# Antibas/eaQHM-analysis-and-synthesis-in-Python

Hardware: AMD Instinct MI355X
Metric: analysis_frames_per_sec (higher is better)
Workload: dtype f64; 1 GPU; synth16k_60s_female_maxAdpt5; samples=960000, fs=16000, ls_frames_per_adaptation=63936, adaptations_executed=5, Kmax=59, track_bytes=906240000, parallelism=instants sharded x1 by LS cost; boundary records all-gathered per adaptation

## Files before the change

eaqhm-analysis-and-synthesis-in-python_amd/csrc/eaqhm_ls_tile.hip:

```cpp
#include "eaqhm_ls_common.h"
#include "eaqhm_ls_chol.h"
#include "eaqhm_ls_a0.h"
#include "eaqhm_ls_tilemap.h"

namespace eaqhm {


#define DIAG_OWNER(jb, nt) ((int)TL_DIAG[nt][jb])
#define TL_THREADS 512
#define TL_WAVES 8
#define TL_CW 8
#define TL_NTMAX 13
#define CI_STRIDE 20
#define CI_NCH 16
#define A0_NS 7
#define A0_M 7

#define TZ_TB 104
#define TZ_NCH 8

__device__ inline void tw_step(d4 (&g)[9], double aR, double aI, double bR, double bI, double nk) {
  const double sA = aR + aI, dB = bI - bR;
  const double naR = nk * aR, naI = nk * aI, nsA = nk * sA;
  const double nbR = nk * bR, nbI = nk * bI, ndB = nk * dB;
  g[0] = __builtin_amdgcn_mfma_f64_16x16x4f64(aR, bR, g[0], 0, 0, 0);
  g[1] = __builtin_amdgcn_mfma_f64_16x16x4f64(aI, bI, g[1], 0, 0, 0);
  g[2] = __builtin_amdgcn_mfma_f64_16x16x4f64(sA, dB, g[2], 0, 0, 0);
  g[3] = __builtin_amdgcn_mfma_f64_16x16x4f64(naR, bR, g[3], 0, 0, 0);
  g[4] = __builtin_amdgcn_mfma_f64_16x16x4f64(naI, bI, g[4], 0, 0, 0);
  g[5] = __builtin_amdgcn_mfma_f64_16x16x4f64(nsA, dB, g[5], 0, 0, 0);
  g[6] = __builtin_amdgcn_mfma_f64_16x16x4f64(naR, nbR, g[6], 0, 0, 0);
  g[7] = __builtin_amdgcn_mfma_f64_16x16x4f64(naI, nbI, g[7], 0, 0, 0);
  g[8] = __builtin_amdgcn_mfma_f64_16x16x4f64(nsA, ndB, g[8], 0, 0, 0);
}

template <int NS, int TW>
__device__ __attribute__((noinline)) void tile_frame(const LsArgs& A, int TS_, int ldx_max_, double* lds, int f_) {
  const int TS = uni(TS_), ldx_max = uni(ldx_max_), f = uni(f_);
  const int tid = threadIdx.x, nt_thr = TL_THREADS;
  const int lane = tid & 63;
  const int wave = __builtin_amdgcn_readfirstlane(tid >> 6);
  double* U = uni(lds);
  double* Xre = U;
  double* Xim = Xre + (size_t)TS * ldx_max;
  const size_t usize_g = (size_t)2 * TS * ldx_max;
  double* ci = U + usize_g;
  unsigned long long* masks = (unsigned long long*)(ci + (size_t)CI_STRIDE * 52);
  double* PanR = U;
  double* PanI = PanR + TL_NTMAX * TL_TILE;
  double* WtR = PanI + TL_NTMAX * TL_TILE;
  double* WtI = WtR + TL_NTMAX * TL_TILE;
  double* LdR = WtI + TL_NTMAX * TL_TILE;
  double* LdI = LdR + TL_TILE;
  double* Dc = LdI + TL_TILE;
  double* Zc = Dc + DG_TILE;
  double* zv = Zc + DG_TILE;
  double* xv = zv + 2 * 16 * TL_NTMAX;
  const size_t usize_c = (size_t)(xv + 32 - U);
  double* xs = U + usize_c;
  double* sh = xs + 4 * uni(A.Kcmax);
  double* win = sh + 16;
  double* sig = win + 64 * CI_NCH;
  double* dorig = sig + 64 * CI_NCH;

  const int Npad = ((uni(A.Nmax) + 63) >> 6) << 6;
  double* Qs = uni(A.scratch) + (size_t)blockIdx.x * (size_t)uni((int)A.scratch_stride);
  double* Rs = Qs + (size_t)Npad * uni(A.nmax);
  const bool seeds = uni((int)(A.any_seed && (*A.any_seed != 0))) != 0;
  const double w1 = uni(2.0 * M_PI / A.fs);
  const int PE = TS / 2;
  const double* sA = uni(A.s);
  const int lcol = lane & 15, lq = lane >> 4;
  unsigned long long* dbg = uni(A.debug);
  unsigned long long t_prev = 0;

  {
    const int n = uni(A.ncol[f]);
    const int Kc = 2 * n + 1, Ms = 2 * Kc + 1;
    const int nt = (Ms + 15) >> 4;
    const int c = uni(A.frame_c[f]), wl = uni(A.frame_wl[f]), inst = uni(A.frame_inst[f]);
    const int N = 2 * wl + 1, mid = wl;
    const int T = (Kc + 16) >> 4;
    const int nb = TW ? T : nt;
    const int ldx = (nb << 4) + ((nb & 1) ? 0 : 16);
    const int npair = T * (T + 1) / 2;
    const int is = 2 * Kc - 16 * (nt - 1);
    const double f0 = uni(A.f0_stale);
    const int* mycols = uni(A.cols) + (size_t)f * uni(A.Kmax);
    const int npairs = mid + 1;

    if (dbg && tid == 0) t_prev = __builtin_amdgcn_s_memtime();
    for (int q = tid; q < 2 * TS * ldx_max; q += nt_thr) Xre[q] = 0.0;
    for (int t = tid; t < N; t += nt_thr) {
      win[t] = window_value(false, t, N);
      sig[t] = sA[(size_t)(c - wl) + t];
    }
    __syncthreads();
    int* gappy = (int*)(masks + (size_t)52 * CI_NCH);
    prepare_slots<CI_STRIDE, TL_WAVES>(A, Qs, Rs, Npad, ci, masks, gappy, mycols, n, N, mid, c, wl, seeds, lane, wave, CI_NCH);
    LS_STAMP(0);

    constexpr int NM3 = (NS <= 7) ? NS : 0;
    d4 accR[NS], accI[NS], acc3[NM3 ? NM3 : 1];
    int tP[NS], tQ[NS];
    bool live[NS];
#pragma unroll
    for (int sl = 0; sl < NS; ++sl) {
      accR[sl] = (d4){0, 0, 0, 0};
      accI[sl] = (d4){0, 0, 0, 0};
      if (sl < NM3) acc3[sl] = (d4){0, 0, 0, 0};
      const int code = TL_MAP[nt][wave][sl];
      live[sl] = code != 0xFF;
      const int P = live[sl] ? (code >> 4) : 0, Q = live[sl] ? (code & 15) : 0;
      tP[sl] = __builtin_amdgcn_readfirstlane(P);
      tQ[sl] = __builtin_amdgcn_readfirstlane(Q);
    }

    constexpr int TWA = TW ? TW : 1;
    d4 g[TWA][9];
    int gI[TWA], gJ[TWA];
    bool glive[TWA];
#pragma unroll
    for (int sl = 0; sl < TWA; ++sl) {
      const int x = wave + 8 * sl;
      glive[sl] = TW && x < npair;
      int I = 0, J = 0;
      if (glive[sl]) tile_of(x, I, J);
      gI[sl] = __builtin_amdgcn_readfirstlane(I);
      gJ[sl] = __builtin_amdgcn_readfirstlane(J);
#pragma unroll
      for (int p = 0; p < 9; ++p) g[sl][p] = (d4){0, 0, 0, 0};
    }

    for (int d0 = 0; d0 < npairs; d0 += PE) {
#pragma clang loop unroll(disable)
      for (int idx = tid; idx < 16 * n; idx += nt_thr) {
        const int el = idx & 15, j = idx >> 4, d = d0 + el;
        const bool act = d <= mid;
        const int u = mid - d - 1, v = mid + d;
        double su = 0, cu = 1, sv, cv;
        double pur = 0, pui = 0, nur = 0, nui = 0, pvr, pvi, nvr, nvi;
        {
          double* cj = ci + j * CI_STRIDE;
          const double* fb = ((const double**)cj)[2];
          const double* ab = ((const double**)cj)[3];
          const int dc = act ? d : mid;
          const double fu1 = fb[mid - dc], fv = fb[mid + dc];
          const double au = ab[(mid - dc - 1 >= 0) ? (mid - dc - 1) : 0], au1 = ab[mid - dc];
          const double av = ab[mid + dc], av1 = ab[(mid + dc + 1 < N) ? (mid + dc + 1) : (N - 1)];
          const double xu = act ? fu1 : 0.0, xv = (act && d >= 1) ? fv : 0.0;
          const double qv = cj[0] + scan16(xv), qu = -(cj[1] + scan16(xu));
          if (el == 15) { cj[0] = qv; cj[1] = -qu; }
          if (!act) continue;
          const double ainv = cj[17], pr = cj[18], pi = cj[19];
          sincos_cw(qu * w1, &su, &cu);
          sincos_cw(qv * w1, &sv, &cv);
          const double eps = 10e-5;
          if (u >= 0) {
            const double ru = (eps + au) * ainv, rv1 = (eps + av1) * ainv;
            pur = ru * cu;                    pui = ru * su;
            nur = rv1 * (cv * pr - sv * pi);  nui = rv1 * (cv * pi + sv * pr);
          }
          const double rv = (eps + av) * ainv, ru1 = (eps + au1) * ainv;
          pvr = rv * cv;                      pvi = rv * sv;
          nvr = ru1 * (cu * pr - su * pi);    nvi = ru1 * (cu * pi + su * pr);
        }
        double* xr = Xre + (2 * el) * ldx;
        double* xi = Xim + (2 * el) * ldx;
        const int cpos = XCOL(n + 1 + j, el), cneg = XCOL(j, el);
        const int spos = XCOL(Kc + n + 1 + j, el), sneg = XCOL(Kc + j, el);
        const double wv = win[v], nv = (double)(v - mid);
        if (u >= 0) {
          const double wu = win[u], nu = (double)(u - mid);
          pur *= wu; pui *= wu; nur *= wu; nui *= wu;
          xr[cpos] = pur;      xi[cpos] = pui;      xr[cneg] = nur;      xi[cneg] = nui;
          if (!TW) { xr[spos] = nu * pur; xi[spos] = nu * pui; xr[sneg] = nu * nur; xi[sneg] = nu * nui; }
        }
        pvr *= wv; pvi *= wv; nvr *= wv; nvi *= wv;
        xr += ldx; xi += ldx;
        xr[cpos] = pvr;      xi[cpos] = pvi;      xr[cneg] = nvr;      xi[cneg] = nvi;
        if (!TW) { xr[spos] = nv * pvr; xi[spos] = nv * pvi; xr[sneg] = nv * nvr; xi[sneg] = nv * nvi; }
      }
      if ((tid & 15) == 0 && (tid >> 4) < TS) {
        const int row = tid >> 4;
        const int d = d0 + (row >> 1);
        const int t = (row & 1) ? (mid + d) : (mid - d - 1);
        const bool ok = (d <= mid) && (t >= 0);
        const double w = ok ? win[t] : 0.0;
        const double sval = ok ? sig[t] : 0.0;
        const double nn = (double)(t - mid);
        const int el = row >> 1;
        double* xr = Xre + row * ldx;
        double* xi = Xim + row * ldx;
        xr[XCOL(n, el)] = w;               xi[XCOL(n, el)] = 0.0;
        if (!TW) {
          xr[XCOL(Kc + n, el)] = w * nn;   xi[XCOL(Kc + n, el)] = 0.0;
        }
        const int scol = TW ? Kc : 2 * Kc;
        xr[XCOL(scol, el)] = w * sval;     xi[XCOL(scol, el)] = 0.0;
      }
      if (d0 + PE > mid) {
        for (int q = tid; q < TS * 16 * nb; q += nt_thr) {
          const int row = q / (16 * nb), col = q - row * (16 * nb);
          const int d = d0 + (row >> 1);
          const int t = (row & 1) ? (mid + d) : (mid - d - 1);
          if (d > mid || t < 0) { Xre[row * ldx + col] = 0.0; Xim[row * ldx + col] = 0.0; }
        }
      }
      LS_STAMP(12);
      __syncthreads();
      LS_STAMP(1);
      const int pcs = (npairs - d0 < PE) ? (npairs - d0) : PE;
      const int ksl = (pcs + 1) >> 1;
      if constexpr (TW > 0) {
#pragma unroll
        for (int sl = 0; sl < TW; ++sl) {
          if (!glive[sl]) continue;
          const int ca = 16 * gI[sl], cb = 16 * gJ[sl];
          int rb = lq * ldx;
          const int sw0 = lcol + (lq >> 1);
          int nk = (lq & 1) ? d0 + (lq >> 1) : -d0 - (lq >> 1) - 1;
          asm volatile("" : "+v"(rb), "+v"(nk));
          const int plane = TS * ldx_max;
          const int kn = (ksl < 8) ? ksl : 8;
#pragma clang loop unroll(disable)
          for (int ks = 0; ks < kn; ++ks) {
            const int sw = (sw0 + 2 * ks) & 15;
            const double aR = Xre[rb + ca + sw], aI = Xre[rb + ca + sw + plane];
            const double bR = Xre[rb + cb + sw], bI = Xre[rb + cb + sw + plane];
            rb += 4 * ldx;
            tw_step(g[sl], aR, aI, bR, bI, (double)nk);
            nk += (lq & 1) ? 2 : -2;
          }
        }
      } else
#pragma unroll
      for (int sl = 0; sl < NS; ++sl) {
        if (!live[sl]) continue;
        const int ca = 16 * tP[sl], cb = 16 * tQ[sl];
        int rb = lq * ldx;
        const int sw0 = lcol + (lq >> 1);
        asm volatile("" : "+v"(rb));
        const int plane = TS * ldx_max;
        if (ksl < 8) {
#pragma clang loop unroll(disable)
          for (int ks = 0; ks < ksl; ++ks) {
            const int sw = (sw0 + 2 * ks) & 15;
            const double aR = Xre[rb + ca + sw], aI = Xre[rb + ca + sw + plane];
            const double bR = Xre[rb + cb + sw], bI = Xre[rb + cb + sw + plane];
            rb += 4 * ldx;
            if (sl < NM3) {
              accR[sl] = __builtin_amdgcn_mfma_f64_16x16x4f64(aR, bR, accR[sl], 0, 0, 0);
              acc3[sl < NM3 ? sl : 0] = __builtin_amdgcn_mfma_f64_16x16x4f64(aI, bI, acc3[sl < NM3 ? sl : 0], 0, 0, 0);
              accI[sl] = __builtin_amdgcn_mfma_f64_16x16x4f64(aR + aI, bI - bR, accI[sl], 0, 0, 0);
            } else {
              accR[sl] = __builtin_amdgcn_mfma_f64_16x16x4f64(aR, bR, accR[sl], 0, 0, 0);
              accI[sl] = __builtin_amdgcn_mfma_f64_16x16x4f64(aR, bI, accI[sl], 0, 0, 0);
              accR[sl] = __builtin_amdgcn_mfma_f64_16x16x4f64(aI, bI, accR[sl], 0, 0, 0);
              accI[sl] = __builtin_amdgcn_mfma_f64_16x16x4f64(-aI, bR, accI[sl], 0, 0, 0);
            }
          }
          continue;
        }
        double aR, aI, bR, bI;
        {
          const int sw = sw0 & 15;
          aR = Xre[rb + ca + sw]; aI = Xre[rb + ca + sw + plane]; bR = Xre[rb + cb + sw]; bI = Xre[rb + cb + sw + plane];
        }
#pragma unroll
        for (int ks = 0; ks < 8; ++ks) {
          double naR = 0, naI = 0, nbR = 0, nbI = 0;
          if (ks < 7) {
            rb += 4 * ldx;
            const int sw = (sw0 + 2 * (ks + 1)) & 15;
            naR = Xre[rb + ca + sw]; naI = Xre[rb + ca + sw + plane]; nbR = Xre[rb + cb + sw]; nbI = Xre[rb + cb + sw + plane];
          }
          __builtin_amdgcn_sched_barrier(0);
          if (sl < NM3) {
            accR[sl] = __builtin_amdgcn_mfma_f64_16x16x4f64(aR, bR, accR[sl], 0, 0, 0);
            acc3[sl < NM3 ? sl : 0] = __builtin_amdgcn_mfma_f64_16x16x4f64(aI, bI, acc3[sl < NM3 ? sl : 0], 0, 0, 0);
            accI[sl] = __builtin_amdgcn_mfma_f64_16x16x4f64(aR + aI, bI - bR, accI[sl], 0, 0, 0);
          } else {
            accR[sl] = __builtin_amdgcn_mfma_f64_16x16x4f64(aR, bR, accR[sl], 0, 0, 0);
            accI[sl] = __builtin_amdgcn_mfma_f64_16x16x4f64(aR, bI, accI[sl], 0, 0, 0);
            accR[sl] = __builtin_amdgcn_mfma_f64_16x16x4f64(aI, bI, accR[sl], 0, 0, 0);
            accI[sl] = __builtin_amdgcn_mfma_f64_16x16x4f64(-aI, bR, accI[sl], 0, 0, 0);
          }
          aR = naR; aI = naI; bR = nbR; bI = nbI;
        }
      }
      __syncthreads();
      LS_STAMP(2);
    }
    if constexpr (TW == 0 && NM3 > 0) {
#pragma unroll
      for (int sl = 0; sl < NM3; ++sl) {
        const d4 p1 = accR[sl], p2 = acc3[sl];
        accR[sl] = p1 + p2;
        accI[sl] = accI[sl] + (p1 - p2);
      }
    }
    if constexpr (TW > 0) {
      double* Gs = Qs;
#pragma unroll
      for (int sl = 0; sl < TWA; ++sl) {
        if (!glive[sl]) continue;
        const int x = wave + 8 * sl;
#pragma unroll
        for (int p = 0; p < 3; ++p) {
          const d4 p1 = g[sl][3 * p], p2 = g[sl][3 * p + 1];
          const d4 re = p1 + p2, im = g[sl][3 * p + 2] + (p1 - p2);
          double* gt = Gs + (size_t)(p * npair + x) * 512;
#pragma unroll
          for (int r = 0; r < 4; ++r) {
            const int o = 2 * (16 * (lq + 4 * r) + lcol);
            gt[o] = re[r]; gt[o + 1] = im[r];
          }
        }
      }
      __syncthreads();
#pragma unroll
      for (int sl = 0; sl < NS; ++sl) {
#pragma unroll
        for (int r = 0; r < 4; ++r) {
          const int R = 16 * tP[sl] + lq + 4 * r, C = 16 * tQ[sl] + lcol;
          const bool pad = !live[sl] || R > 2 * Kc || C > 2 * Kc;
          const bool rs = R >= Kc && R < 2 * Kc, cs = C >= Kc && C < 2 * Kc;
          const int a = (R == 2 * Kc) ? Kc : rs ? R - Kc : R, b = (C == 2 * Kc) ? Kc : cs ? C - Kc : C;
          const int p = (int)rs + (int)cs;
          const bool lo = (a >> 4) >= (b >> 4);
          const int I = lo ? (a >> 4) : (b >> 4), J = lo ? (b >> 4) : (a >> 4);
          const int i = lo ? (a & 15) : (b & 15), j = lo ? (b & 15) : (a & 15);
          double vr = 0.0, vi = 0.0;
          if (!pad) {
            const double2 v = *(const double2*)(Gs + (size_t)(p * npair + I * (I + 1) / 2 + J) * 512 + 2 * (16 * i + j));
            vr = v.x; vi = lo ? v.y : -v.y;
          }
          accR[sl][r] = vr; accI[sl][r] = vi;
        }
      }
      LS_STAMP(2);
    }

    {
#pragma unroll
      for (int sl = 0; sl < NS; ++sl) {
        if (!live[sl] || tP[sl] != nt - 1) continue;
#pragma unroll
        for (int r = 0; r < 4; ++r) {
          const int row = lq + 4 * r, col = lcol;
          const bool pad = (row > is) || (tQ[sl] == nt - 1 && col > is);
          if (pad) {
            accR[sl][r] = (tQ[sl] == nt - 1 && row == col) ? 1.0 : 0.0;
            accI[sl][r] = 0.0;
          }
        }
      }
#pragma unroll
      for (int sl = 0; sl < NS; ++sl) {
        if (!live[sl] || tP[sl] != tQ[sl]) continue;
#pragma unroll
        for (int r = 0; r < 4; ++r)
          if (lq + 4 * r == lcol) dorig[16 * tP[sl] + lcol] = accR[sl][r];
      }
      double* post = Dc;
      double* dumpD = Dc + DGP_DOUBLES;
      double* zs = dumpD + 128;
      int* dflag = (int*)(zs + 256);
      if (tid == 0) *dflag = 0;
      __syncthreads();
#define TRAILING_UPDATE(sl)                                                                         \
  {                                                                                                 \
    const double* ar = PanR + tP[sl] * TL_TILE;                                                     \
    const double* ai = PanI + tP[sl] * TL_TILE;                                                     \
    const double* br = PanR + tQ[sl] * TL_TILE;                                                     \
    const double* bi = PanI + tQ[sl] * TL_TILE;                                                     \
       \
       \
    d4 p1 = (d4){0, 0, 0, 0}, p2 = (d4){0, 0, 0, 0};                                                \
    _Pragma("unroll") for (int ks = 0; ks < 4; ++ks) {                                              \
      const int o = (4 * ks + lq) * TL_LD + lcol;                                                   \
      const double aR = ar[o], aI = ai[o], lR = br[o], lI = bi[o];                                  \
      p1 = __builtin_amdgcn_mfma_f64_16x16x4f64(aR, lR, p1, 0, 0, 0);                               \
      p2 = __builtin_amdgcn_mfma_f64_16x16x4f64(aI, lI, p2, 0, 0, 0);                               \
      accI[sl] = __builtin_amdgcn_mfma_f64_16x16x4f64(aR + aI, lI - lR, accI[sl], 0, 0, 0);         \
    }                                                                                               \
    accR[sl] = accR[sl] - (p1 + p2);                                                                \
    accI[sl] = accI[sl] + (p1 - p2);                                                                \
  }
      for (int jb = 0; jb < nt; ++jb) {
        d4 Rt = (d4){0, 0, 0, 0}, It = (d4){0, 0, 0, 0};
        bool mine = false;
#pragma unroll
        for (int sl = 0; sl < NS; ++sl) {
          if (!live[sl] || tP[sl] != jb || tQ[sl] != jb) continue;
          if (jb > 0) TRAILING_UPDATE(sl)
          Rt = accR[sl]; It = accI[sl];
          mine = true;
        }
        if (mine) {
          unsigned long long td0 = 0;
          unsigned long long* tlast = (unsigned long long*)(dflag + 2);
          const bool tdiag = dbg && uni(A.debug_diag);
          if (tdiag) td0 = __builtin_amdgcn_s_memtime();
          diag_D(Rt, It, post, nullptr, dflag, 16 * jb, dumpD, LdR, LdI, jb == nt - 1);
          if (tdiag && lane == 0) {
            const unsigned long long td1 = __builtin_amdgcn_s_memtime();
            atomicAdd(dbg + 9, td1 - td0);
            if (jb > 0) { atomicAdd(dbg + 11, td0 - *tlast); atomicAdd(dbg + 14, 1ull); }
            atomicAdd(dbg + 13, 1ull);
            *tlast = td1;
          }
        }
        LS_STAMP(10);
        if (jb > 0) {
#pragma unroll
          for (int sl = 0; sl < NS; ++sl) {
            if (!live[sl] || tQ[sl] < jb || (tP[sl] == jb && tQ[sl] == jb)) continue;
            TRAILING_UPDATE(sl)
          }
        }
        LS_STAMP(8);
        if (!mine && wave == (int)TL_HELP[nt][jb])
          diag_Z(post, dflag, 16 * jb, zs, WtR + jb * TL_TILE, WtI + jb * TL_TILE, dorig + 16 * jb,
                 (jb == nt - 1) ? is : 16, uni(A.fault));
        __syncthreads();
        LS_STAMP(6);
#pragma unroll
        for (int sl = 0; sl < NS; ++sl) {
          if (!live[sl] || tQ[sl] != jb || tP[sl] == jb) continue;
          double* tr = PanR + tP[sl] * TL_TILE;
          double* ti = PanI + tP[sl] * TL_TILE;
#pragma unroll
          for (int r = 0; r < 4; ++r) {
            tr[lcol * TL_LD + lq + 4 * r] = accR[sl][r];
            ti[lcol * TL_LD + lq + 4 * r] = accI[sl][r];
          }
          __builtin_amdgcn_wave_barrier();
          d4 p1 = (d4){0, 0, 0, 0}, p2 = (d4){0, 0, 0, 0}, p3 = (d4){0, 0, 0, 0};
          const double* wr = WtR + jb * TL_TILE;
          const double* wi = WtI + jb * TL_TILE;
#pragma unroll
          for (int ks = 0; ks < 4; ++ks) {
            const int o = (4 * ks + lq) * TL_LD + lcol;
            const double aR = tr[o], aI = ti[o], bR = wr[o], bI = wi[o];
            p1 = __builtin_amdgcn_mfma_f64_16x16x4f64(aR, bR, p1, 0, 0, 0);
            p2 = __builtin_amdgcn_mfma_f64_16x16x4f64(aI, bI, p2, 0, 0, 0);
            p3 = __builtin_amdgcn_mfma_f64_16x16x4f64(aR + aI, bR + bI, p3, 0, 0, 0);
          }
          const d4 xr = p1 - p2, xi = p3 - (p1 + p2);
          accR[sl] = xr; accI[sl] = xi;
          __builtin_amdgcn_wave_barrier();
#pragma unroll
          for (int r = 0; r < 4; ++r) {
            tr[lcol * TL_LD + lq + 4 * r] = xr[r];
            ti[lcol * TL_LD + lq + 4 * r] = xi[r];
          }
        }
        LS_STAMP(7);
        __syncthreads();
      }
#undef TRAILING_UPDATE
      __syncthreads();
      LS_STAMP(3);

#pragma unroll
      for (int sl = 0; sl < NS; ++sl) {
        if (!live[sl] || tP[sl] != nt - 1 || tQ[sl] == nt - 1) continue;
        if (lq == (is & 3)) {
#pragma unroll
          for (int r = 0; r < 4; ++r)
            if (r == (is >> 2)) {
              zv[2 * (16 * tQ[sl] + lcol)] = accR[sl][r];
              zv[2 * (16 * tQ[sl] + lcol) + 1] = -accI[sl][r];
            }
        }
      }
      if (tid < 16) {
        const bool ok = tid < is;
        zv[2 * (16 * (nt - 1) + tid)] = ok ? LdR[is * TL_LD + tid] : 0.0;
        zv[2 * (16 * (nt - 1) + tid) + 1] = ok ? -LdI[is * TL_LD + tid] : 0.0;
      }
      for (int q = tid; q < 4 * Kc; q += nt_thr) xs[q] = 0.0;
      __syncthreads();
      for (int P = nt - 1; P >= 0; --P) {
        if (tid < 256) {
          const int i = tid >> 4, k = tid & 15;
          double xr = 0, xi = 0;
          if (k >= i) {
            const double wr = WtR[P * TL_TILE + i * TL_LD + k], wi = WtI[P * TL_TILE + i * TL_LD + k];
            const double zr = zv[2 * (16 * P + k)], zi = zv[2 * (16 * P + k) + 1];
            xr = wr * zr - wi * zi;
            xi = wr * zi + wi * zr;
          }
#pragma unroll
          for (int o = 8; o > 0; o >>= 1) { xr += __shfl_xor(xr, o); xi += __shfl_xor(xi, o); }
          if (k == 0) {
            xv[2 * i] = xr; xv[2 * i + 1] = xi;
            const int q = 16 * P + i;
            if (q < 2 * Kc) { xs[2 * q] = xr; xs[2 * q + 1] = xi; }
          }
        }
        __syncthreads();
#pragma unroll
        for (int sl = 0; sl < NS; ++sl) {
          if (!live[sl] || tP[sl] != P || tQ[sl] == P) continue;
          double sr = 0, si = 0;
#pragma unroll
          for (int r = 0; r < 4; ++r) {
            const double xr = xv[2 * (lq + 4 * r)], xi = xv[2 * (lq + 4 * r) + 1];
            const double lr = accR[sl][r], li = accI[sl][r];
            sr += lr * xr + li * xi;
            si += lr * xi - li * xr;
          }
          sr += __shfl_xor(sr, 16); si += __shfl_xor(si, 16);
          sr += __shfl_xor(sr, 32); si += __shfl_xor(si, 32);
          if (lq == 0) {
            zv[2 * (16 * tQ[sl] + lcol)] -= sr;
            zv[2 * (16 * tQ[sl] + lcol) + 1] -= si;
          }
        }
        __syncthreads();
      }
      LS_STAMP(4);
    }

    write_record(A, xs, sh, mycols, f, n, inst, c, f0, seeds);
    LS_STAMP(5);
  }
}

__device__ inline int frame_class(int n) {
  const int nt = (2 * (2 * n + 1) + 1 + 15) >> 4;
  return nt <= 8 ? 0 : nt == 9 ? 1 : nt == 10 ? 2 : nt == 11 ? 3 : nt == 12 ? 4 : nt <= TL_NTMAX ? 5 : LS_BIG_CLASS;
}
extern "C" __global__ void __launch_bounds__(256) eaqhm_ls_classify_kernel(LsArgs A) {
  const int f = blockIdx.x * blockDim.x + threadIdx.x, lane = threadIdx.x & 63;
  int cl = (f < A.n_frames) ? frame_class((A.mode == 0) ? A.frame_K[f] : A.ncol[f]) : -1;
  if (f < A.n_frames) {
    if (!frame_window_ok(A, A.frame_c[f], A.frame_wl[f])) { cl = -1; atomicAdd(A.fault + 2, 1); }
  }
  if (A.mode == 1 && cl >= 0) {
    const long long c = A.frame_c[f], wl = A.frame_wl[f];
    const long long lo = (c - wl - 1 > 0) ? (c - wl - 1) : 0;
    for (long long ch = lo >> 10; ch <= ((c + wl) >> 10); ++ch) A.zflag[ch] = 1;
  }
  for (int c = 0; c < LS_NCLS; ++c) {
    const unsigned long long m = __ballot(cl == c);
    if (m == 0ull) continue;
    int base = 0;
    if (lane == __ffsll((long long)m) - 1) base = atomicAdd(A.cls + c, __popcll(m));
    base = __shfl(base, __ffsll((long long)m) - 1);
    if (cl == c) A.cls[16 + (size_t)c * A.n_frames + base + __popcll(m & ((1ull << lane) - 1ull))] = f;
  }
}

extern "C" __global__ void __launch_bounds__(256) eaqhm_ls_zero_prefix_kernel(const double* __restrict__ fm, long long Lt,
                                                                              long long t_lo, int ch0, int zchunks,
                                                                              const unsigned char* __restrict__ zflag,
                                                                              unsigned short* __restrict__ zloc,
                                                                              int* __restrict__ ztot) {
  __shared__ int wsum[4];
  const int k = blockIdx.y, ch = ch0 + blockIdx.x, tid = threadIdx.x, lane = tid & 63, wave = tid >> 6;
  if (!zflag[ch]) return;
  const long long base = (long long)ch << 10;
  int run = 0;
  for (int p = 0; p < 4; ++p) {
    const long long t = base + 256 * p + tid;
    const bool in = t >= t_lo && t < t_lo + Lt;
    const bool z = in && (fm[(size_t)k * Lt + t] == 0.0);
    const unsigned long long m = __ballot(z);
    const int incl = __popcll(m & ((lane == 63) ? ~0ull : ((1ull << (lane + 1)) - 1ull)));
    if (lane == 0) wsum[wave] = __popcll(m);
    __syncthreads();
    int off = 0, tot = 0;
#pragma unroll
    for (int w = 0; w < 4; ++w) { const int v = wsum[w]; tot += v; if (w < wave) off += v; }
    if (in) zloc[(size_t)k * Lt + t] = (unsigned short)(run + off + incl);
    run += tot;
    __syncthreads();
  }
  if (tid == 0) ztot[(size_t)k * zchunks + ch] = run;
}

extern "C" __global__ void __launch_bounds__(TL_THREADS) eaqhm_ls_tile_kernel(LsArgs A, int TS, int ldx_max) {
  extern __shared__ __attribute__((aligned(16))) double lds[];
  __shared__ int nxt;
#define RUN_CLASS(NSV, TWV, C)                                                             \
  for (;;) {                                                                             \
    if (threadIdx.x == 0) nxt = atomicAdd(A.cls + 8 + C, 1);                             \
    __syncthreads();                                                                     \
    const int item = nxt;                                                                \
    __syncthreads();                                                                     \
    if (item >= A.cls[C]) break;                                                         \
    if (A.mode == 0) a0_frame<A0_NS, A0_M, 2>(A, lds, A.cls[16 + (size_t)C * A.n_frames + item], TZ_TB, TZ_NCH, 520, 64 * CI_NCH);                          \
    else tile_frame<NSV, TWV>(A, TS, ldx_max, lds, A.cls[16 + (size_t)C * A.n_frames + item]);          \
  }
  RUN_CLASS(12, 0, 5)
  RUN_CLASS(10, 0, 4)
  RUN_CLASS(9, 0, 3)
  RUN_CLASS(7, 2, 2)
  RUN_CLASS(6, 2, 1)
  RUN_CLASS(5, 2, 0)
#undef RUN_CLASS
}

#define TL_LDS_LIMIT (159 * 1024)
static size_t tl_usize_c() {
  return (size_t)4 * TL_NTMAX * TL_TILE + 2 * TL_TILE + 2 * DG_TILE + 2 * 16 * TL_NTMAX + 32;
}
static size_t tl_usize_g(int TS, int ldx_max) { return (size_t)2 * TS * ldx_max + (size_t)CI_STRIDE * 52 + 52 * CI_NCH + 32; }
static size_t tl_lds_doubles(int Kcmax, int TS, int ldx_max) {
  const size_t c = tl_usize_c(), g = tl_usize_g(TS, ldx_max);
  return (c > g ? c : g) + 4 * (size_t)Kcmax + 16 + 2 * 64 * CI_NCH + 16 * TL_NTMAX;
}

bool ls_tile_applicable(int Kcmax, int Nmax) {
  return Nmax <= 64 * CI_NCH && tl_lds_doubles(Kcmax, 32, 16 * TL_NTMAX + 16) * sizeof(double) <= TL_LDS_LIMIT;
}

size_t ls_tile_scratch_stride(int nmax, int Nmax) {
  const size_t Npad = (size_t)((Nmax + 63) >> 6) << 6;
  const size_t bridged = 2 * Npad * nmax, gram = (size_t)3 * 21 * 512;
  return ((bridged > gram ? bridged : gram) + 15) & ~(size_t)15;
}

int launch_ls_prepass(eaqhm_ctx* ctx, LsArgs A, long long track_t0) {
  hipLaunchKernelGGL(eaqhm_ls_classify_kernel, dim3((A.n_frames + 255) / 256), dim3(256), 0, ctx->stream, A);
  HIP_TRY(ctx, hipGetLastError());
  if (A.mode == 1) {
    const int ch0 = (int)(track_t0 >> 10), ch1 = (int)((track_t0 + A.Lt - 1) >> 10);
    hipLaunchKernelGGL(eaqhm_ls_zero_prefix_kernel, dim3(ch1 - ch0 + 1, A.Kmax), dim3(256), 0, ctx->stream, A.fm_cur, A.Lt,
                       track_t0, ch0, A.zchunks, A.zflag, (unsigned short*)A.zloc, (int*)A.ztot);
    HIP_TRY(ctx, hipGetLastError());
  }
  return EAQHM_OK;
}

int launch_ls_tile(eaqhm_ctx* ctx, LsArgs A, int grid) {
  const int Kcmax = A.Kcmax;
  const int ldx_max = 16 * TL_NTMAX + 16;
  const int TS = 32;
  const size_t lds_bytes = tl_lds_doubles(Kcmax, TS, ldx_max) * sizeof(double);
  if (lds_bytes > TL_LDS_LIMIT) return ctx->fail(EAQHM_EINVAL, "eaqhm_ls_batch: LDS budget exceeded (tile variant)");
  if (a0_lds_doubles(A0_M, 2, TZ_TB, TZ_NCH, 520, 64 * CI_NCH, Kcmax) * sizeof(double) > lds_bytes)
    return ctx->fail(EAQHM_EINVAL, "eaqhm_ls_batch: LDS budget exceeded (adaptation 0, tile variant)");
  HIP_TRY(ctx, hipFuncSetAttribute((const void*)eaqhm_ls_tile_kernel, hipFuncAttributeMaxDynamicSharedMemorySize, (int)lds_bytes));
  hipLaunchKernelGGL(eaqhm_ls_tile_kernel, dim3(grid), dim3(TL_THREADS), lds_bytes, ctx->stream, A, TS, ldx_max);
  HIP_TRY(ctx, hipGetLastError());
  return EAQHM_OK;
}

}
```

Baseline: 1.457 million frames/s.

## Balance three-weight Gram tiles across waves with a deal table and single-weight units

Replaces the fixed round-robin assignment of Gram tile pairs to waves with a precomputed deal table. The table hands each wave whole three-weight tiles plus individual weight units (one of three moment accumulators), so the MFMA work per wave is more even. It also enables the three-weight Gram path for the larger classes (NS 9 and 10), which previously used the plain tile map. The cost is more code-size and register pressure from the extra accumulator sets, some duplicate LDS loads for the single units, and a dependence on the table being correct for each tile count.

After: 1.445 million frames/s. About the same (-0.8%).

```diff
diff --git a/eaqhm-analysis-and-synthesis-in-python_amd/csrc/eaqhm_ls_tile.hip b/eaqhm-analysis-and-synthesis-in-python_amd/csrc/eaqhm_ls_tile.hip
--- a/eaqhm-analysis-and-synthesis-in-python_amd/csrc/eaqhm_ls_tile.hip
+++ b/eaqhm-analysis-and-synthesis-in-python_amd/csrc/eaqhm_ls_tile.hip
@@ -2,6 +2,7 @@
 #include "eaqhm_ls_chol.h"
 #include "eaqhm_ls_a0.h"
 #include "eaqhm_ls_tilemap.h"
+#include "eaqhm_ls_twdeal.h"
 
 namespace eaqhm {
 
@@ -34,7 +35,14 @@
   g[8] = __builtin_amdgcn_mfma_f64_16x16x4f64(nsA, ndB, g[8], 0, 0, 0);
 }
 
-template <int NS, int TW>
+__device__ inline void tw_unit_step(d4 (&h)[3], double aR, double aI, double bR, double bI, double s1, double s2) {
+  const double sA = aR + aI, dB = bI - bR;
+  h[0] = __builtin_amdgcn_mfma_f64_16x16x4f64(s1 * aR, s2 * bR, h[0], 0, 0, 0);
+  h[1] = __builtin_amdgcn_mfma_f64_16x16x4f64(s1 * aI, s2 * bI, h[1], 0, 0, 0);
+  h[2] = __builtin_amdgcn_mfma_f64_16x16x4f64(s1 * sA, s2 * dB, h[2], 0, 0, 0);
+}
+
+template <int NS, int TW, int TU>
 __device__ __attribute__((noinline)) void tile_frame(const LsArgs& A, int TS_, int ldx_max_, double* lds, int f_) {
   const int TS = uni(TS_), ldx_max = uni(ldx_max_), f = uni(f_);
   const int tid = threadIdx.x, nt_thr = TL_THREADS;
@@ -116,20 +124,37 @@
       tQ[sl] = __builtin_amdgcn_readfirstlane(Q);
     }
 
-    constexpr int TWA = TW ? TW : 1;
-    d4 g[TWA][9];
-    int gI[TWA], gJ[TWA];
-    bool glive[TWA];
+    constexpr int TWA = TW ? TW : 1, TUA = TU ? TU : 1;
+    static_assert(TW > 0 || TU == 0, "single units belong to the three-weight form");
+    d4 g[TWA][9], h[TUA][3];
+    int gI[TWA], gJ[TWA], gX[TWA], hI[TUA], hJ[TUA], hX[TUA], hP[TUA];
+    bool glive[TWA], hlive[TUA];
 #pragma unroll
     for (int sl = 0; sl < TWA; ++sl) {
-      const int x = wave + 8 * sl;
-      glive[sl] = TW && x < npair;
+      const int code = TW ? (int)TW_DEAL[TW ? T : 0][wave][3 * sl] : 0xFF;
+      glive[sl] = code != 0xFF;
+      const int x = glive[sl] ? (code >> 2) : 0;
       int I = 0, J = 0;
-      if (glive[sl]) tile_of(x, I, J);
+      tile_of(x, I, J);
+      gX[sl] = __builtin_amdgcn_readfirstlane(x);
       gI[sl] = __builtin_amdgcn_readfirstlane(I);
       gJ[sl] = __builtin_amdgcn_readfirstlane(J);
 #pragma unroll
       for (int p = 0; p < 9; ++p) g[sl][p] = (d4){0, 0, 0, 0};
+    }
+#pragma unroll
+    for (int su = 0; su < TUA; ++su) {
+      const int code = TU ? (int)TW_DEAL[TU ? T : 0][wave][3 * TW + su] : 0xFF;
+      hlive[su] = code != 0xFF;
+      const int x = hlive[su] ? (code >> 2) : 0;
+      int I = 0, J = 0;
+      tile_of(x, I, J);
+      hX[su] = __builtin_amdgcn_readfirstlane(x);
+      hI[su] = __builtin_amdgcn_readfirstlane(I);
+      hJ[su] = __builtin_amdgcn_readfirstlane(J);
+      hP[su] = __builtin_amdgcn_readfirstlane(hlive[su] ? (code & 3) : 0);
+#pragma unroll
+      for (int p = 0; p < 3; ++p) h[su][p] = (d4){0, 0, 0, 0};
     }
 
     for (int d0 = 0; d0 < npairs; d0 += PE) {
@@ -233,6 +258,35 @@
             nk += (lq & 1) ? 2 : -2;
           }
         }
+        bool hany = false;
+#pragma unroll
+        for (int su = 0; su < TU; ++su) hany = hany || hlive[su];
+        if (TU > 0 && hany) {
+          int rb = lq * ldx;
+          const int sw0 = lcol + (lq >> 1);
+          int nk = (lq & 1) ? d0 + (lq >> 1) : -d0 - (lq >> 1) - 1;
+          asm volatile("" : "+v"(rb), "+v"(nk));
+          const int plane = TS * ldx_max;
+          const int kn = (ksl < 8) ? ksl : 8;
+#pragma clang loop unroll(disable)
+          for (int ks = 0; ks < kn; ++ks) {
+            const int sw = (sw0 + 2 * ks) & 15;
+            const double nd = (double)nk;
+            double aR = 0, aI = 0, bR = 0, bI = 0;
+#pragma unroll
+            for (int su = 0; su < TU; ++su) {
+              if (!hlive[su]) continue;
+              if (su == 0 || !hlive[su - 1] || hX[su] != hX[su - 1]) {
+                const int ca = 16 * hI[su], cb = 16 * hJ[su];
+                aR = Xre[rb + ca + sw]; aI = Xre[rb + ca + sw + plane];
+                bR = Xre[rb + cb + sw]; bI = Xre[rb + cb + sw + plane];
+              }
+              tw_unit_step(h[su], aR, aI, bR, bI, hP[su] >= 1 ? nd : 1.0, hP[su] == 2 ? nd : 1.0);
+            }
+            rb += 4 * ldx;
+            nk += (lq & 1) ? 2 : -2;
+          }
+        }
       } else
 #pragma unroll
       for (int sl = 0; sl < NS; ++sl) {
@@ -305,7 +359,7 @@
 #pragma unroll
       for (int sl = 0; sl < TWA; ++sl) {
         if (!glive[sl]) continue;
-        const int x = wave + 8 * sl;
+        const int x = gX[sl];
 #pragma unroll
         for (int p = 0; p < 3; ++p) {
           const d4 p1 = g[sl][3 * p], p2 = g[sl][3 * p + 1];
@@ -316,6 +370,18 @@
             const int o = 2 * (16 * (lq + 4 * r) + lcol);
             gt[o] = re[r]; gt[o + 1] = im[r];
           }
+        }
+      }
+#pragma unroll
+      for (int su = 0; su < TU; ++su) {
+        if (!hlive[su]) continue;
+        const d4 p1 = h[su][0], p2 = h[su][1];
+        const d4 re = p1 + p2, im = h[su][2] + (p1 - p2);
+        double* gt = Gs + (size_t)(hP[su] * npair + hX[su]) * 512;
+#pragma unroll
+        for (int r = 0; r < 4; ++r) {
+          const int o = 2 * (16 * (lq + 4 * r) + lcol);
+          gt[o] = re[r]; gt[o + 1] = im[r];
         }
       }
       __syncthreads();
@@ -586,7 +652,7 @@
 extern "C" __global__ void __launch_bounds__(TL_THREADS) eaqhm_ls_tile_kernel(LsArgs A, int TS, int ldx_max) {
   extern __shared__ __attribute__((aligned(16))) double lds[];
   __shared__ int nxt;
-#define RUN_CLASS(NSV, TWV, C)                                                             \
+#define RUN_CLASS(NSV, TWV, TUV, C)                                                             \
   for (;;) {                                                                             \
     if (threadIdx.x == 0) nxt = atomicAdd(A.cls + 8 + C, 1);                             \
     __syncthreads();                                                                     \
@@ -594,15 +660,17 @@
     __syncthreads();                                                                     \
     if (item >= A.cls[C]) break;                                                         \
     if (A.mode == 0) a0_frame<A0_NS, A0_M, 2>(A, lds, A.cls[16 + (size_t)C * A.n_frames + item], TZ_TB, TZ_NCH, 520, 64 * CI_NCH);                          \
-    else tile_frame<NSV, TWV>(A, TS, ldx_max, lds, A.cls[16 + (size_t)C * A.n_frames + item]);          \
+    else tile_frame<NSV, TWV, TUV>(A, TS, ldx_max, lds, A.cls[16 + (size_t)C * A.n_frames + item]);          \
   }
-  RUN_CLASS(12, 0, 5)
-  RUN_CLASS(10, 0, 4)
-  RUN_CLASS(9, 0, 3)
-  RUN_CLASS(7, 2, 2)
-  RUN_CLASS(6, 2, 1)
-  RUN_CLASS(5, 2, 0)
+  RUN_CLASS(12, 0, 0, 5)
+  RUN_CLASS(10, 2, 2, 4)
+  RUN_CLASS(9, 2, 2, 3)
+  RUN_CLASS(7, 2, 2, 2)
+  RUN_CLASS(6, 2, 2, 1)
+  RUN_CLASS(5, 1, 1, 0)
 #undef RUN_CLASS
+  static_assert(TW_WHOLE[1] == 1 && TW_WHOLE[4] == 1 && TW_SINGLE[1] == 1 && TW_SINGLE[4] == 1, "class 0");
+  static_assert(TW_WHOLE[5] == 2 && TW_SINGLE[5] == 2 && TW_WHOLE[6] == 2 && TW_SINGLE[6] == 2, "classes 1 - 4");
 }
 
 #define TL_LDS_LIMIT (159 * 1024)
diff --git a/eaqhm-analysis-and-synthesis-in-python_amd/csrc/eaqhm_ls_twdeal.h b/eaqhm-analysis-and-synthesis-in-python_amd/csrc/eaqhm_ls_twdeal.h
--- /dev/null
+++ b/eaqhm-analysis-and-synthesis-in-python_amd/csrc/eaqhm_ls_twdeal.h
@@ -0,0 +1,14 @@
+#pragma once
+namespace eaqhm {
+constexpr unsigned char TW_WHOLE[7] = {0, 1, 1, 1, 1, 2, 2};
+constexpr unsigned char TW_SINGLE[7] = {0, 1, 1, 1, 1, 2, 2};
+__device__ const unsigned char TW_DEAL[7][8][8] = {
+  {{0xFF, 0xFF, 0xFF, 0xFF, 0xFF, 0xFF, 0xFF, 0xFF}, {0xFF, 0xFF, 0xFF, 0xFF, 0xFF, 0xFF, 0xFF, 0xFF}, {0xFF, 0xFF, 0xFF, 0xFF, 0xFF, 0xFF, 0xFF, 0xFF}, {0xFF, 0xFF, 0xFF, 0xFF, 0xFF, 0xFF, 0xFF, 0xFF}, {0xFF, 0xFF, 0xFF, 0xFF, 0xFF, 0xFF, 0xFF, 0xFF}, {0xFF, 0xFF, 0xFF, 0xFF, 0xFF, 0xFF, 0xFF, 0xFF}, {0xFF, 0xFF, 0xFF, 0xFF, 0xFF, 0xFF, 0xFF, 0xFF}, {0xFF, 0xFF, 0xFF, 0xFF, 0xFF, 0xFF, 0xFF, 0xFF}},
+  {{0xFF, 0xFF, 0xFF, 0x00, 0xFF, 0xFF, 0xFF, 0xFF}, {0xFF, 0xFF, 0xFF, 0x01, 0xFF, 0xFF, 0xFF, 0xFF}, {0xFF, 0xFF, 0xFF, 0x02, 0xFF, 0xFF, 0xFF, 0xFF}, {0xFF, 0xFF, 0xFF, 0xFF, 0xFF, 0xFF, 0xFF, 0xFF}, {0xFF, 0xFF, 0xFF, 0xFF, 0xFF, 0xFF, 0xFF, 0xFF}, {0xFF, 0xFF, 0xFF, 0xFF, 0xFF, 0xFF, 0xFF, 0xFF}, {0xFF, 0xFF, 0xFF, 0xFF, 0xFF, 0xFF, 0xFF, 0xFF}, {0xFF, 0xFF, 0xFF, 0xFF, 0xFF, 0xFF, 0xFF, 0xFF}},
+  {{0x00, 0x01, 0x02, 0xFF, 0xFF, 0xFF, 0xFF, 0xFF}, {0xFF, 0xFF, 0xFF, 0x04, 0xFF, 0xFF, 0xFF, 0xFF}, {0xFF, 0xFF, 0xFF, 0x06, 0xFF, 0xFF, 0xFF, 0xFF}, {0xFF, 0xFF, 0xFF, 0x09, 0xFF, 0xFF, 0xFF, 0xFF}, {0xFF, 0xFF, 0xFF, 0xFF, 0xFF, 0xFF, 0xFF, 0xFF}, {0xFF, 0xFF, 0xFF, 0x05, 0xFF, 0xFF, 0xFF, 0xFF}, {0xFF, 0xFF, 0xFF, 0x08, 0xFF, 0xFF, 0xFF, 0xFF}, {0xFF, 0xFF, 0xFF, 0x0A, 0xFF, 0xFF, 0xFF, 0xFF}},
+  {{0x00, 0x01, 0x02, 0x11, 0xFF, 0xFF, 0xFF, 0xFF}, {0x04, 0x05, 0x06, 0x14, 0xFF, 0xFF, 0xFF, 0xFF}, {0x08, 0x09, 0x0A, 0xFF, 0xFF, 0xFF, 0xFF, 0xFF}, {0x0C, 0x0D, 0x0E, 0xFF, 0xFF, 0xFF, 0xFF, 0xFF}, {0xFF, 0xFF, 0xFF, 0x10, 0xFF, 0xFF, 0xFF, 0xFF}, {0xFF, 0xFF, 0xFF, 0x12, 0xFF, 0xFF, 0xFF, 0xFF}, {0xFF, 0xFF, 0xFF, 0x15, 0xFF, 0xFF, 0xFF, 0xFF}, {0xFF, 0xFF, 0xFF, 0x16, 0xFF, 0xFF, 0xFF, 0xFF}},
+  {{0x00, 0x01, 0x02, 0x20, 0xFF, 0xFF, 0xFF, 0xFF}, {0x08, 0x09, 0x0A, 0x22, 0xFF, 0xFF, 0xFF, 0xFF}, {0x10, 0x11, 0x12, 0x25, 0xFF, 0xFF, 0xFF, 0xFF}, {0x18, 0x19, 0x1A, 0x26, 0xFF, 0xFF, 0xFF, 0xFF}, {0x04, 0x05, 0x06, 0x21, 0xFF, 0xFF, 0xFF, 0xFF}, {0x0C, 0x0D, 0x0E, 0x24, 0xFF, 0xFF, 0xFF, 0xFF}, {0x14, 0x15, 0x16, 0xFF, 0xFF, 0xFF, 0xFF, 0xFF}, {0x1C, 0x1D, 0x1E, 0xFF, 0xFF, 0xFF, 0xFF, 0xFF}},
+  {{0x00, 0x01, 0x02, 0x04, 0x05, 0x06, 0xFF, 0xFF}, {0x10, 0x11, 0x12, 0x14, 0x15, 0x16, 0xFF, 0xFF}, {0x1C, 0x1D, 0x1E, 0x20, 0x21, 0x22, 0xFF, 0xFF}, {0x28, 0x29, 0x2A, 0x2C, 0x2D, 0x2E, 0xFF, 0xFF}, {0x08, 0x09, 0x0A, 0x0C, 0x0D, 0x0E, 0xFF, 0xFF}, {0x18, 0x19, 0x1A, 0xFF, 0xFF, 0xFF, 0x34, 0x35}, {0x24, 0x25, 0x26, 0xFF, 0xFF, 0xFF, 0x36, 0x38}, {0x30, 0x31, 0x32, 0xFF, 0xFF, 0xFF, 0x39, 0x3A}},
+  {{0x00, 0x01, 0x02, 0x04, 0x05, 0x06, 0x40, 0x41}, {0x10, 0x11, 0x12, 0x14, 0x15, 0x16, 0x45, 0x46}, {0x20, 0x21, 0x22, 0x24, 0x25, 0x26, 0x4A, 0x4C}, {0x30, 0x31, 0x32, 0x34, 0x35, 0x36, 0x50, 0x51}, {0x08, 0x09, 0x0A, 0x0C, 0x0D, 0x0E, 0x42, 0x44}, {0x18, 0x19, 0x1A, 0x1C, 0x1D, 0x1E, 0x48, 0x49}, {0x28, 0x29, 0x2A, 0x2C, 0x2D, 0x2E, 0x4D, 0x4E}, {0x38, 0x39, 0x3A, 0x3C, 0x3D, 0x3E, 0x52, 0xFF}},
+};
+}
```
